# jscanvic/Scale-Equivariant-Imaging

Measured on AMD Instinct MI355X. Metric: training images/sec (256x256 crops), proposed-loss deblur, higher is better.
Workload: dtype bf16; 1 GPU; BASELINE configs[1]: deblurring Gaussian_R2 noise=5, proposed loss (SURE + scale-EI), 256x256 pairs cropped to 48 in Loss.forward, ConvolutionalModel hidden=32 scales=5; parameters=645063043, batch_per_gpu=32, global_batch=32, parallelism=dp1

## Files before the change

### include/sei_hip.h

```cpp
#ifndef SEI_HIP_H
#define SEI_HIP_H

#include <stddef.h>
#include <stdint.h>

#ifdef __cplusplus
extern "C" {
#endif

#define SEI_OK 0
#define SEI_ERR_BAD_ARG 10001
#define SEI_ERR_TOO_LARGE 10002


#define SEI_ABI_VERSION 12
int sei_abi_version(void);
int sei_build_target(char *name, int n);

int sei_event_create(void **event);
int sei_event_destroy(void *event);
int sei_event_record_external(void *event, void *stream);
int sei_stream_wait_event(void *stream, void *event);

int sei_graph_node_counts(void *graph, int *kernel_nodes, int *all_nodes);
// ... 221 lines not shown
int sei_sepmap2_small(const float *x, void *y, int out_bf16, int B, int Hi, int Wi, int Ho, int Wo, int C,
                      const float *L1, const float *R1, const float *L2, const float *R2, void *stream);
int sei_sepmap2_bf16_out16(const float *x, uint16_t *y16, int B, int Hi, int Wi, int Ho, int Wo, int C,
                           const uint16_t *packed, void *stream);

int sei_sepmap2(const float *x, float *y, int B, int Hi, int Wi, int Ho, int Wo, int C,
                const float *L1, const float *R1, const float *L2, const float *R2, float *work,
                size_t work_floats, void *stream);
int sei_sepmap2_bf16(const float *x, float *y, int B, int Hi, int Wi, int Ho, int Wo, int C, const uint16_t *packed,
                     void *stream);
int sei_sepmap2_bf16_pack(const float *L1, const float *R1, const float *L2, const float *R2, uint16_t *packed, int Hi,
                          int Wi, int Ho, int Wo, void *stream);
size_t sei_sepmap2_bf16_eligible(int B, int Hi, int Wi, int Ho, int Wo, int C);
size_t sei_sepmap2_bf16_pack_elems(int Hi, int Wi, int Ho, int Wo);
size_t sei_sepmap2_big_eligible(int B, int Hi, int Wi, int Ho, int Wo, int C);
size_t sei_sepmap2_big_pack_elems(int Hi, int Wi, int Ho, int Wo);
size_t sei_sepmap2_big_work_elems(int B, int Hi, int Wi, int Ho, int Wo, int C);
int sei_sepmap2_big_pack(const float *L1, const float *R1, const float *L2, const float *R2, uint16_t *packed,
                         int Hi, int Wi, int Ho, int Wo, void *stream);
int sei_sepmap2_big(const float *x, float *y, int B, int Hi, int Wi, int Ho, int Wo, int C, const uint16_t *packed,
                    uint16_t *work, void *stream);
int sei_sepmap2_packed(const float *x, float *y, int B, int Hi, int Wi, int Ho, int Wo, int C,
                       const float *RW, const float *LH, float *work, size_t work_floats, void *stream);

int sei_colsum_f32(const float *X, float *out, size_t M, int N, void *stream);
int sei_colsum_weighted_f32(const float *X, const float *row_weight, float *out, size_t M, int N, void *stream);

size_t sei_mlp_fused_eligible(long long M, int C);
int sei_mlp_fused_fwd(const uint16_t *h2, const uint16_t *W2, const float *b2, const uint16_t *W3, const float *b3,
                      const float *x, float res_scale, float *out, int M, int C, void *stream);
int sei_mlp_fused_bwd(const float *go, const uint16_t *h2, const uint16_t *W2, const float *b2, const uint16_t *W3T,
                      const uint16_t *W2T, float *gh2, uint16_t *go16, uint16_t *h4, uint16_t *gh3, int M, int C,
                      void *stream);

int sei_swin_attn_fwd(const float *qkv, const float *table, float *out, int B, int H, int W, int heads,
                      int head_dim, int shift, float scale, void *stream);
int sei_swin_attn_bwd(const float *qkv, const float *table, const float *dout, float *dqkv, float *dtable,
                      int B, int H, int W, int heads, int head_dim, int shift, float scale, void *stream);
int sei_swin_attn_fwd_bf16(const uint16_t *qkv, const float *table, uint16_t *out, float *lse, int B, int H, int W,
                           int heads, int shift, float scale, void *stream);
int sei_swin_attn_bwd_bf16(const uint16_t *qkv, const float *table, const uint16_t *out, const float *lse,
                           const uint16_t *dout, uint16_t *dqkv, float *dtable, int B, int H, int W, int heads,
                           int shift, float scale, void *stream);
int sei_pad_nhwc(const float *x, float *xp, int B, int H, int W, int C, int guard_rows, void *stream);
int sei_unpad_nhwc(const float *xp, const float *res, float *y, int B, int H, int W, int C, int act, void *stream);
int sei_rowscale(const float *x, const float *row_scale, const float *leaky_gate, float *y, size_t M, int N,
                 void *stream);

int sei_pack(const float *src, const int *map, void *dst, size_t n, int to_bf16, void *stream);
int sei_unpack_add(const float *src, const int *map, float *dst, size_t n, void *stream);
int sei_ln_fwd_bf16_pad(const float *x, const float *gamma, const float *beta, uint16_t *y, float *mean,
                        float *rstd, size_t rows, int C, int ldy, float eps, int ones_col, void *stream);
size_t sei_swin_partials_floats(int C);
int sei_ln_bwd_pad(const float *x, const float *gamma, const float *mean, const float *rstd, const float *gy,
                   const float *res, float *gx, float *ggamma, float *gbeta, size_t rows, int C, int ldg,
                   float *work, size_t work_floats, void *stream);
int sei_cast_pad_bf16(const float *x, const float *row_scale, uint16_t *y, float *colsum, size_t rows, int C,
                      int ldy, float *work, size_t work_floats, void *stream);
int sei_pad_nhwc_bf16(const float *x, uint16_t *xp, int B, int H, int W, int C, int Cp, int guard_rows, void *stream);
int sei_pad_nhwc_bf16_ones(const float *x, uint16_t *xp, int B, int H, int W, int C, int Cp, int guard_rows, int ones_col,
                           void *stream);
int sei_gemm_bf16nt_conv(const uint16_t *Ap, int cin_pad, const int *row_off9, const uint16_t *B, int ldb,
                         float *D32, uint16_t *D16, int M, int N, int epilogue, const float *bias, void *stream);
int sei_gemm_bf16nt_conv_unpad(const uint16_t *Ap, int cin_pad, const int *row_off9, const uint16_t *B, int ldb, float *y,
                               const float *res, int Bimg, int H, int W, int N, const float *bias, int act, void *stream);

// ... 141 lines not shown
```

### scale-equivariant-imaging_amd/_native.py

```python
import ctypes
import os

import torch

_HERE = os.path.dirname(os.path.abspath(__file__))
LIB_PATH = os.environ.get("SEI_HIP_LIBRARY") or os.path.join(_HERE, "libsei_hip.so")

SEI_REDUCE_BLOCKS = 256

_c = ctypes
_P, _I, _F, _Z, _L = _c.c_void_p, _c.c_int, _c.c_float, _c.c_size_t, _c.c_longlong

SIGNATURES = {
    "sei_abi_version": [],
    "sei_event_create": [_P],
    "sei_event_destroy": [_P],
    "sei_event_record_external": [_P, _P],
    "sei_stream_wait_event": [_P, _P],
    "sei_graph_node_counts": [_P, _P, _P],
    "sei_build_target": [_c.c_char_p, _I],
    "sei_blur_sep_circ": [_P, _P, _P, _P, _I, _I, _I, _I, _I, _I, _P],
    "sei_blur_dense_circ": [_P, _P, _P, _I, _I, _I, _I, _I, _I, _P],
    "sei_blur_dense_pad": [_P, _P, _P, _I, _I, _I, _I, _I, _I, _I, _P, _P],
    "sei_circ_filter_sep": [_P, _P, _P, _P, _I, _I, _I, _P],
# ... 50 lines not shown
    "sei_ln_fwd_bf16": [_P, _P, _P, _P, _P, _P, _Z, _I, _F, _P],
    "sei_colsum_bf16": [_P, _P, _Z, _I, _P],
    "sei_split_bf16x2": [_P, _P, _Z, _P],
    "sei_split_bf16x3": [_P, _P, _Z, _I, _P],
    "sei_gelu_f32": [_P, _P, _Z, _P],
    "sei_mul_dgelu_f32": [_P, _P, _Z, _P],
    "sei_cast_transpose_bf16": [_P, _I, _P, _P, _I, _I, _I, _P, _P],
    "sei_cast_bf16_colsum_weighted": [_P, _P, _P, _P, _I, _I, _P],
    "sei_cast_bf16_colsum_parts": [_P, _P, _P, _P, _I, _I, _P],
    "sei_gemm_bf16nt": [_P, _I, _I, _P, _I, _I, _P, _P, _I, _I, _I, _I, _P, _P, _P, _P, _P],
    "sei_gemm_bf16nt_colsum": [_P, _I, _I, _P, _I, _I, _P, _I, _I, _I, _I, _P, _P, _P],
    "sei_gemm_bf16nt_ws": [_P, _I, _I, _P, _I, _I, _P, _P, _I, _I, _I, _I, _P, _P, _P, _P, _P, _P, _Z, _I, _I, _I, _P],
    "sei_fold_many": [_P, _I, _P],
    "sei_transpose_bf16_many": [_P, _I, _P],
    "sei_gemm_bf16nt_dw2": [_P, _P, _I, _P, _P, _I, _P, _I, _I, _I, _I, _I, _P],
    "sei_gemm_bf16nt_ex": [_P, _I, _I, _P, _I, _I, _P, _P, _I, _I, _I, _I, _P, _P, _P, _P, _I, _I, _P],
    "sei_gemm_bf16nt_dw2_ex": [_P, _P, _I, _P, _P, _I, _P, _I, _I, _I, _I, _I, _I, _P],
    "sei_gemm_bf16nt_dw2_adam": [_P, _P, _I, _P, _P, _I, _P, _P, _P, _P, _P, _I, _I, _I, _I, _P],
    "sei_gemm_bf16nt_dw2_adam_ex": [_P, _P, _I, _P, _P, _I, _P, _P, _P, _P, _P, _I, _I, _I, _I, _I, _P],
    "sei_gemm_bf16nt_dw2_bf16out": [_P, _P, _I, _P, _P, _I, _P, _I, _I, _I, _I, _P],
    "sei_gemm_bf16nt_dw2_taps": [_P, _P, _I, _P, _P, _I, _P, _I, _I, _I, _I, _I, _I, _P, _L, _P],
    "sei_sepmap2": [_P, _P, _I, _I, _I, _I, _I, _I, _P, _P, _P, _P, _P, _Z, _P],
    "sei_sepmap2_big_pack": [_P, _P, _P, _P, _P, _I, _I, _I, _I, _P],
    "sei_sepmap2_big": [_P, _P, _I, _I, _I, _I, _I, _I, _P, _P, _P],
    "sei_sepmap2_packed": [_P, _P, _I, _I, _I, _I, _I, _I, _P, _P, _P, _Z, _P],
    "sei_sepmap2_bf16": [_P, _P, _I, _I, _I, _I, _I, _I, _P, _P],
    "sei_sepmap2_bf16_pack": [_P, _P, _P, _P, _P, _I, _I, _I, _I, _P],
    "sei_sepmap2_small": [_P, _P, _I, _I, _I, _I, _I, _I, _I, _P, _P, _P, _P, _P],
    "sei_sepmap2_bf16_out16": [_P, _P, _I, _I, _I, _I, _I, _I, _P, _P],
    "sei_colsum_f32": [_P, _P, _Z, _I, _P],
    "sei_colsum_weighted_f32": [_P, _P, _P, _Z, _I, _P],
    "sei_mlp_fused_fwd": [_P, _P, _P, _P, _P, _P, _F, _P, _I, _I, _P],
    "sei_mlp_fused_bwd": [_P, _P, _P, _P, _P, _P, _P, _P, _P, _P, _I, _I, _P],
    "sei_swin_attn_fwd": [_P, _P, _P, _I, _I, _I, _I, _I, _I, _F, _P],
    "sei_swin_attn_bwd": [_P, _P, _P, _P, _P, _I, _I, _I, _I, _I, _I, _F, _P],
    "sei_swin_attn_fwd_bf16": [_P, _P, _P, _P, _I, _I, _I, _I, _I, _F, _P],
    "sei_swin_attn_bwd_bf16": [_P, _P, _P, _P, _P, _P, _P, _I, _I, _I, _I, _I, _F, _P],
    "sei_pad_nhwc": [_P, _P, _I, _I, _I, _I, _I, _P],
    "sei_unpad_nhwc": [_P, _P, _P, _I, _I, _I, _I, _I, _P],
    "sei_rowscale": [_P, _P, _P, _P, _Z, _I, _P],
    "sei_pack": [_P, _P, _P, _Z, _I, _P],
    "sei_unpack_add": [_P, _P, _P, _Z, _P],
    "sei_ln_fwd_bf16_pad": [_P, _P, _P, _P, _P, _P, _Z, _I, _I, _F, _I, _P],
    "sei_ln_bwd_pad": [_P, _P, _P, _P, _P, _P, _P, _P, _P, _Z, _I, _I, _P, _Z, _P],
    "sei_cast_pad_bf16": [_P, _P, _P, _P, _Z, _I, _I, _P, _Z, _P],
    "sei_pad_nhwc_bf16": [_P, _P, _I, _I, _I, _I, _I, _I, _P],
    "sei_pad_nhwc_bf16_ones": [_P, _P, _I, _I, _I, _I, _I, _I, _I, _P],
    "sei_gemm_bf16nt_conv": [_P, _I, _P, _P, _I, _P, _P, _I, _I, _I, _P, _P],
    "sei_gemm_bf16nt_conv_unpad": [_P, _I, _P, _P, _I, _P, _P, _I, _I, _I, _I, _P, _I, _P],
    "sei_rowgemm_bf16": [_P, _I, _P, _I, _P, _I, _P, _I, _L, _I, _I, _I, _I, _P, _P, _P, _I, _P],
    "sei_rowgemm_lnbwd_bf16": [_P, _I, _P, _I, _L, _I, _P, _P, _P, _P, _P, _P, _I, _P, _P, _P, _P, _I, _P, _P, _Z, _P],
    "sei_rowgemm_dgelu_bf16": [_P, _I, _P, _I, _P, _I, _P, _I, _P, _I, _P, _I, _L, _I, _I, _P],
    "sei_rowgemm_ln_bf16": [_P, _I, _P, _I, _L, _I, _I, _P, _P, _P, _P, _P, _P, _F, _I, _P, _I, _P, _P, _P],
    "sei_rowgemm_gelu_bf16": [_P, _I, _P, _I, _P, _I, _P, _I, _L, _I, _I, _I, _P],
    "sei_tokgrad_bf16_blocks": [_P, _I, _L, _L, _P],
    "sei_tokgrad_bf16": [_P, _P, _I, _P, _P, _I, _P, _I, _I, _I, _L, _L, _P],
    "sei_dwstream_bf16_jobs": [_P, _I, _P],
    "sei_adam_fused": [_P, _P, _I, _P, _P, _Z, _F, _F, _F, _F, _F, _I, _F, _P, _P],
    "sei_adam_scalars": [_F, _F, _F, _F, _F, _I, _P, _P],
    "sei_adam_scalars_to_device": [_F, _F, _F, _F, _F, _I, _P, _P],
    "sei_sgd_fused": [_P, _P, _P, _P, _Z, _Z, _F, _F, _P, _P, _I, _P],
    "sei_sgd_penalty_finish": [_P, _Z, _P, _P],
    "sei_adam_anchor_fused": [_P, _P, _P, _P, _P, _P, _Z, _Z, _F, _F, _F, _F, _F, _I, _F, _P, _P, _I, _P],
    "sei_drunet_conv3x3": [_P, _P, _I, _I, _I, _I, _I, _I, _P, _P, _P, _P, _P],
    "sei_drunet_conv3x3_ex": [_P, _P, _I, _I, _I, _I, _I, _I, _P, _P, _P, _P, _I, _P],
    "sei_drunet_down": [_P, _P, _I, _I, _I, _I, _I, _P, _P, _P],
# ... 45 lines not shown


class TransposeJob(_c.Structure):
    _fields_ = [("src", _P), ("dst", _P), ("R", _I), ("C", _I)]


TRANSPOSE_MAX_JOBS = 16

CG_STATE_WORDS, CG_DONE, CG_ITERATIONS = 8, 3, 4


SIZE_QUERIES = {
    "sei_blur_sep_circ_lds": [_I, _I, _I, _I],
    "sei_blur_dense_pad_work_floats": [_I, _I, _I, _I, _I, _I, _I],
    "sei_resample_sepband_lds": [_I, _I, _I, _I, _I, _I, _I, _I],
    "sei_proposed_draws_max_numel": [],
    "sei_ssim_luma_work_floats": [_I, _I, _I],
    "sei_lpips_work_floats": [_I, _I, _I],
    "sei_tv_prox_work_floats": [_I, _I, _I],
    "sei_dip_work_floats": [_I, _I, _I, _I],
    "sei_dwconv7_bwd_weight_workspace": [_I, _I, _I, _I],
    "sei_dwconv7_bwd_weight_workspace_ex": [_I, _I, _I, _I, _I],
    "sei_ln_bwd_workspace": [_Z, _I],
    "sei_dwconv7_ln_fwd_launches": [_I, _I, _I, _I],
    "sei_sepmap2_bf16_eligible": [_I, _I, _I, _I, _I, _I],
    "sei_sepmap2_bf16_pack_elems": [_I, _I, _I, _I],
    "sei_sepmap2_big_eligible": [_I, _I, _I, _I, _I, _I],
    "sei_sepmap2_big_pack_elems": [_I, _I, _I, _I],
    "sei_sepmap2_big_work_elems": [_I, _I, _I, _I, _I, _I],
    "sei_swin_partials_floats": [_I],
    "sei_tokgrad_bf16_eligible": [_I, _I, _I, _I, _L, _L],
    "sei_dwstream_bf16_eligible": [_I, _I, _I, _I, _L, _L],
    "sei_mlp_fused_eligible": [_L, _I],
    "sei_rowgemm_bf16_eligible": [_L, _I, _I, _I, _I],
    "sei_rowgemm_lnbwd_bf16_eligible": [_L, _I, _I],
    "sei_rowgemm_lnbwd_work_floats": [_I],
    "sei_ln_bwd_part_offset": [_Z, _I],
    "sei_ln_bwd_part_count": [_Z, _I],
    "sei_rowgemm_dgelu_bf16_eligible": [_L, _I, _I],
    "sei_rowgemm_ln_bf16_eligible": [_L, _I, _I],
    "sei_gemm_bf16nt_plan": [_I, _I, _I, _I, _I, _I, _I, _I],
    "sei_gemm_bf16nt_plan_ws": [_I, _I, _I, _I, _I, _I, _I, _I, _Z],
    "sei_gemm_bf16nt_dw2_adam_plan": [_I, _I, _I, _I, _I],
    "sei_conv3x3_bwd_weight_parts_count": [_I, _I, _I, _I, _I, _I, _I],
    "sei_sepmap2_small_eligible": [_I, _I, _I, _I, _I, _I],
    "sei_cast_bf16_colsum_parts_count": [_I, _I],
    "sei_sgd_partials": [_Z, _Z, _I],
    "sei_adam_anchor_partials": [_Z, _Z, _I],
    "sei_drunet_work_bytes": [_I, _I, _I],
    "sei_cg_partials": [_Z],
    "sei_dps_partials": [_I, _Z],
    "sei_bm3d_ref_blocks": [_I, _I, _I],
}
ABI_VERSION = 12


class NativeLibraryError(RuntimeError):
    pass


def lib():
    global _lib
    if _lib is None:
        if not os.path.exists(LIB_PATH):
            raise NativeLibraryError(
                f"{LIB_PATH} is missing: build it with `make -C {os.path.join(_HERE, 'csrc')}` "
# ... 147 lines not shown
```

### scale-equivariant-imaging_amd/csrc/mlp128.hip

```cpp
#include "sei_common.h"

namespace {

constexpr int WAVES = 9, NT = 64 * WAVES, PX = 16 * WAVES;
constexpr int NSTAGE = 4;

template <int C>
__device__ __forceinline__ void issue_rows(char *dst, const unsigned short *m, int ht, int p, int lane) {
    int r, c;
    if constexpr (C == 128) { r = 4 * p + (lane >> 4); c = (lane & 15) ^ (r & 15); }
    else { r = 16 * p + (lane >> 2); c = (lane & 3) ^ ((-(r >> 2)) & 3); }
    __builtin_amdgcn_global_load_lds((glb_void *)(m + (size_t)(32 * ht + r) * C + 8 * c), (lds_void *)(dst + p * 1024), 16, 0, 0);
}
template <int C>
__device__ __forceinline__ void issue_cols(char *dst, const unsigned short *m, int ht, int p, int lane) {
    const int r = 16 * p + (lane >> 2), c = (lane & 3) ^ ((r >> 2) & 3);
    __builtin_amdgcn_global_load_lds((glb_void *)(m + (size_t)r * (4 * C) + 32 * ht + 8 * c), (lds_void *)(dst + p * 1024), 16, 0, 0);
}
template <int C>
__device__ __forceinline__ bf16x8 rows_frag(const char *img, int t, int ks, int l16, int lg) {
    const int r = 16 * t + l16, c = 4 * ks + lg;
    if constexpr (C == 128) return *reinterpret_cast<const bf16x8 *>(img + (16 * r + (c ^ (r & 15))) * 16);
    else return *reinterpret_cast<const bf16x8 *>(img + (4 * r + (c ^ ((-(r >> 2)) & 3))) * 16);
}
// ... 201 lines not shown
            for (int r = 0; r < 4; ++r) {
                const float h3 = hT[t][r] + bias[t][r];
                float cdf, pdf;
                sei_phi_pdf_bf16out(h3, cdf, pdf);
                const float gv = gT[t][r] * fmaf(h3, pdf, cdf);
                gT[t][r] = gv;
                a4[r] = (__bf16)(h3 * cdf);
                g4[r] = (__bf16)gv;
            }
            *reinterpret_cast<bf16x4 *>(h4p + 32 * ht + 16 * t) = a4;
            *reinterpret_cast<bf16x4 *>(g3p + 32 * ht + 16 * t) = g4;
        }
        const bf16x8 a = pack_tiles(gT[0], gT[1]);
#pragma unroll
        for (int cb = 0; cb < CB; ++cb) acc[cb] = sei_mfma16(a, wb[cb], acc[cb]);
    }
    sei_wait_vmcnt<0>();
    __syncthreads();

    constexpr int QR = C / 4, ITS = 16 * QR / 64;
    float *patch = reinterpret_cast<float *>(smem) + wave * 16 * LDP;
#pragma unroll
    for (int cb = 0; cb < CB; ++cb)
#pragma unroll
        for (int r = 0; r < 4; ++r) patch[(4 * lg + r) * LDP + 16 * cb + l16] = acc[cb][r];
    asm volatile("s_waitcnt lgkmcnt(0)" ::: "memory");
#pragma unroll
    for (int it = 0; it < ITS; ++it) {
        const int idx = it * 64 + lane, p = idx / QR, q = idx % QR;
        *reinterpret_cast<f32x4 *>(gh2 + (px0 + p) * C + 4 * q) = *reinterpret_cast<const f32x4 *>(patch + p * LDP + 4 * q);
    }
}

}

bool sei_mlp128_eligible(int M, int Cc) { return (Cc == 128 || Cc == 32) && M > 0 && M % 144 == 0; }

int sei_mlp128_fwd_launch(const uint16_t *h2, const uint16_t *W2, const float *b2, const uint16_t *W3, const float *b3,
                          const float *x, float res_scale, float *out, int M, int Cc, hipStream_t s) {
    if (Cc == 128)
        hipLaunchKernelGGL(mlp128_fwd_kernel<128>, dim3((unsigned)(M / 144)), dim3(NT), 0, s, h2, W2, b2, W3, b3, x, res_scale, out);
    else
        hipLaunchKernelGGL(mlp128_fwd_kernel<32>, dim3((unsigned)(M / 144)), dim3(NT), 0, s, h2, W2, b2, W3, b3, x, res_scale, out);
    return sei_launch_status();
}

int sei_mlp128_bwd_launch(const float *go, const uint16_t *h2, const uint16_t *W2, const float *b2, const uint16_t *W3T,
                          const uint16_t *W2T, float *gh2, uint16_t *go16, uint16_t *h4, uint16_t *gh3, int M, int Cc,
                          hipStream_t s) {
    if (Cc == 128)
        hipLaunchKernelGGL(mlp128_bwd_kernel<128>, dim3((unsigned)(M / 144)), dim3(NT), 0, s, go, h2, W2, b2, W3T, W2T, gh2,
                           go16, h4, gh3);
    else
        hipLaunchKernelGGL(mlp128_bwd_kernel<32>, dim3((unsigned)(M / 144)), dim3(NT), 0, s, go, h2, W2, b2, W3T, W2T, gh2,
                           go16, h4, gh3);
    return sei_launch_status();
}
```

### scale-equivariant-imaging_amd/csrc/mlp_fused.hip

```cpp
#include "sei_common.h"

namespace {

__device__ __forceinline__ int acc_row(int reg, int lane) { return (reg & 3) + 8 * (reg >> 2) + 4 * (lane >> 5); }
__device__ __forceinline__ bf16x8 acc_frag(const f32x16 &x, int s) {
    bf16x8 a;
#pragma unroll
    for (int e = 0; e < 8; ++e) a[e] = (__bf16)x[8 * s + e];
    return a;
}

constexpr int WAVES = 4, THREADS = 64 * WAVES;

template <int C>
struct Slices {
    static constexpr int ROW_PITCH = C * 2 + 16, COL_PITCH = 72;
    static constexpr int ROW_BYTES = 32 * ROW_PITCH, COL_BYTES = C * COL_PITCH;
    static constexpr int ROW_PIECES = 32 * C / 8, COL_PIECES = C * 4;
    static constexpr int ROW_PER_THREAD = (ROW_PIECES + THREADS - 1) / THREADS;
    static constexpr int COL_PER_THREAD = (COL_PIECES + THREADS - 1) / THREADS;
};

template <int C>
__device__ __forceinline__ void row_slice_load(const unsigned short *m, int ht, uint4 (&r)[Slices<C>::ROW_PER_THREAD]) {
// ... 292 lines not shown
                           x, res_scale, out, M);
    else
        hipLaunchKernelGGL((mlp_fwd_kernel<128, 1>), dim3(mlp_grid(M, 32 * WAVES)), dim3(THREADS), 0, s, h2, W2, b2, W3, b3,
                           x, res_scale, out, M);
    return sei_launch_status();
}

extern "C" int sei_mlp_fused_bwd(const float *go, const uint16_t *h2, const uint16_t *W2, const float *b2,
                                 const uint16_t *W3T, const uint16_t *W2T, float *gh2, uint16_t *go16, uint16_t *h4,
                                 uint16_t *gh3, int M, int C, void *stream) {
    SEI_REQUIRE(go && h2 && W2 && b2 && W3T && W2T && gh2 && go16 && h4 && gh3 && M > 0 && (C == 32 || C == 128));
    SEI_REQUIRE((((uintptr_t)go | (uintptr_t)h2 | (uintptr_t)W2 | (uintptr_t)W3T | (uintptr_t)W2T | (uintptr_t)go16) & 15) == 0 &&
                (((uintptr_t)h4 | (uintptr_t)gh3) & 7) == 0);
    hipStream_t s = (hipStream_t)stream;
    if (sei_mlp128_eligible(M, C)) {
        SEI_REQUIRE((((uintptr_t)gh2 | (uintptr_t)go) & 15) == 0);
        return sei_mlp128_bwd_launch(go, h2, W2, b2, W3T, W2T, gh2, go16, h4, gh3, M, C, s);
    }
    if (const int main = mlp128_main(M, C)) {
        SEI_REQUIRE((((uintptr_t)gh2 | (uintptr_t)go) & 15) == 0);
        if (int rc = sei_mlp128_bwd_launch(go, h2, W2, b2, W3T, W2T, gh2, go16, h4, gh3, main, C, s)) return rc;
        const size_t o = (size_t)main * C;
        go += o; h2 += o; gh2 += o; go16 += o; h4 += 4 * o; gh3 += 4 * o;
        M -= main;
    }
    if (C == 32)
        hipLaunchKernelGGL((mlp_bwd_kernel<32, 2>), dim3(mlp_grid(M, 64 * WAVES)), dim3(THREADS), 0, s, go, h2, W2, b2, W3T,
                           W2T, gh2, go16, h4, gh3, M);
    else
        hipLaunchKernelGGL((mlp_bwd_kernel<128, 1>), dim3(mlp_grid(M, 32 * WAVES)), dim3(THREADS), 0, s, go, h2, W2, b2,
                           W3T, W2T, gh2, go16, h4, gh3, M);
    return sei_launch_status();
}
```

### scale-equivariant-imaging_amd/csrc/sei_common.h

```cpp
#pragma once
#include <hip/hip_runtime.h>
#include <stdint.h>

#include "../../include/sei_hip.h"
#include "sei_mfma.h"

#define SEI_WAVE 64

typedef __attribute__((address_space(3))) void lds_void;
typedef __attribute__((address_space(1))) const void glb_void;

#define SEI_REQUIRE(cond) \
    do {                  \
        if (!(cond)) return SEI_ERR_BAD_ARG; \
    } while (0)

static inline int sei_launch_status() { return (int)hipGetLastError(); }

static inline size_t sei_ceil_div(size_t a, size_t b) { return (a + b - 1) / b; }

static inline unsigned sei_capped_grid(size_t work_items, int per_block, unsigned cap) {
    size_t g = sei_ceil_div(work_items, (size_t)per_block);
    if (g < 1) g = 1;
    if (g > cap) g = cap;
// ... 62 lines not shown
    poly = fmaf(poly, t, -0.284496736f);
    poly = fmaf(poly, t, 0.254829592f);
    const float q = 0.5f * poly * t * e;
    cdf = x >= 0.f ? 1.0f - q : q;
    pdf = 0.39894228040143267794f * e;
}
__device__ __forceinline__ float sei_gelu_bf16out(float x) {
    float cdf, pdf;
    sei_phi_pdf_bf16out(x, cdf, pdf);
    return x * cdf;
}
__device__ __forceinline__ float sei_dgelu_bf16out(float x) {
    float cdf, pdf;
    sei_phi_pdf_bf16out(x, cdf, pdf);
    return fmaf(x, pdf, cdf);
}

__device__ __forceinline__ float sei_adam_element(float pi, float gi, float &mi, float &vi, float beta1, float beta2,
                                              float eps, float wd, float step_size, float inv_bc2_sqrt) {
    if (wd != 0.f) gi = fmaf(wd, pi, gi);
    mi = mi + (gi - mi) * (1.f - beta1);
    vi = fmaf(beta2, vi, (1.f - beta2) * gi * gi);
    const float denom = sqrtf(vi) * inv_bc2_sqrt + eps;
    return pi - step_size * (mi / denom);
}


bool sei_mlp128_eligible(int M, int C);
int sei_mlp128_fwd_launch(const uint16_t *h2, const uint16_t *W2, const float *b2, const uint16_t *W3, const float *b3,
                          const float *x, float res_scale, float *out, int M, int C, hipStream_t s);
int sei_mlp128_bwd_launch(const float *go, const uint16_t *h2, const uint16_t *W2, const float *b2, const uint16_t *W3T,
                          const uint16_t *W2T, float *gh2, uint16_t *go16, uint16_t *h4, uint16_t *gh3, int M, int C,
                          hipStream_t s);

int sei_dwconv7_pipe_launch(const float *x, const float *w, const float *bias, const float *res, float res_scale,
                            float *y, int B, int H, int W, int C, int flip, hipStream_t s);
bool sei_dwconv7_pipe_eligible(const float *x, const float *w, int B, int H, int W, int C);
bool sei_dwconv7_ln_fused_eligible(const float *x, const float *w, int B, int H, int W, int C);
int sei_dwconv7_ln_fused_launch(const float *x, const float *w, const float *bias, const float *gamma,
                                const float *beta, float *h1, void *h2, int out16, float *mean, float *rstd, int B, int H,
                                int W, int C, float eps, hipStream_t s);

__attribute__((visibility("hidden"))) int sei_fold_now(const SeiFoldJob &job, hipStream_t s);
static inline SeiFoldJob sei_fold_job(int kind, const float *part, int groups, int ncol, int split, float *a, float *b,
                                      float *c) {
    SeiFoldJob J{};
    J.a = a; J.b = b; J.c = c; J.ncol = ncol; J.split = split; J.kind = kind; J.nseg = 1;
    J.part[0] = part; J.groups[0] = groups;
    return J;
}
enum { SEI_CG_FOLD_RS = 0, SEI_CG_FOLD_PAP = 1, SEI_CG_FOLD_RS_NEW = 2 };
__attribute__((visibility("hidden"))) int sei_fold_cg(const float *part, int groups, SeiCgState *state, int target, float tol,
                                                      hipStream_t s);
```

### scale-equivariant-imaging_amd/models/_ops.py

```python
import os

import torch

import _native as N
from . import _mats, _wgrad
from ._gemm import (EPI_ACCUM, EPI_BIAS, EPI_BIAS_GELU, EPI_BIAS_RES, EPI_BIAS_ROWSCALE, EPI_MUL_DGELU, EPI_NONE,
                    SPLITK_COUNTER_BYTES, SPLITK_WS_MIB, SPLITK_WS_STREAMS, _SPLITK_WS, _gemm_call, _in_forward_mode,
                    compute_dtype_scope, gemm, gemm_mixed, gemm_nt16, gemm_x3, get_compute_dtype, joint_rows,
                    own_splitk_workspace, profile_gemms, release_splitk_workspace, reset_splitk_counters, set_compute_dtype,
                    splitk_workspace)
from ._joint import JointCtx, _NotJoint, joint_ctx, walk_backward
from ._shadow import (ShadowState, _new_plain_state, _transposed16, _transposed16_cached, plain_shadow_is_current,
                      refresh_plain_shadow, set_stale_masters, shadow, split_x2, weights_updated)
from ._wgrad import (_state_for, begin_step, colsum16_into, defer_fold, direct_bf16_launches, flush_weight_grads,
                     fused_adam_launches, merged_weight_grads, note_forward, register_gradient_range,
                     set_direct_bf16_grads, set_fused_adam, set_weight_grad_merging, set_weight_grad_milestone, state_of,
                     weight_grad16, weight_grad16_group, weight_grad_views)

LN_EPS = 1e-6


def grad_of(p):
    if p.grad is None:
        view = getattr(p, "_sei_grad_view", None)
# ... 398 lines not shown
        ctx.params = (w1, b1, gamma, beta, w2, b2, w3, b3)
        ctx.twice = twice
        return out.view(B, H, W, C)

    @_in_forward_mode
    def backward(ctx, go):
        if ctx.fused:
            return ConvBlockFn16._backward_fused(ctx, go)
        x, h1, mean, rstd, h2, h3, h4 = ctx.saved_tensors
        w1, b1, gamma, beta, w2, b2, w3, b3 = ctx.params
        B, H, W, C = x.shape
        M = B * H * W
        go = go.contiguous()
        go2 = go.view(M, C)
        go16 = cast16(go2, colsum_into_=grad_of(b3))
        gh3 = torch.empty((M, 4 * C), dtype=torch.bfloat16, device=x.device)
        gemm_nt16(go16, shadow(w3), M, 4 * C, C, EPI_MUL_DGELU, out16=gh3, R1=h3, b_rmajor=True, colsum=grad_of(b2))
        weight_grad16(go16, h4, grad_of(w3).view(C, 4 * C))
        gh2 = torch.empty((M, C), dtype=torch.float32, device=x.device)
        gemm_nt16(gh3, shadow(w2), M, C, 4 * C, EPI_NONE, out32=gh2, b_rmajor=True)
        weight_grad16(gh3, h2, grad_of(w2).view(4 * C, C))
        return _convblock_tail(ctx, x, h1, mean, rstd, gh2, go)

    @staticmethod
    def _backward_fused(ctx, go):
        x, h1, mean, rstd, h2 = ctx.saved_tensors
        w1, b1, gamma, beta, w2, b2, w3, b3 = ctx.params
        B, H, W, C = x.shape
        M = B * H * W
        go = go.contiguous()
        dev = x.device
        w2_16, w3_16 = shadow(w2), shadow(w3)
        gh2 = torch.empty((M, C), dtype=torch.float32, device=dev)
        go16 = torch.empty((M, C), dtype=torch.bfloat16, device=dev)
        h4 = torch.empty((M, 4 * C), dtype=torch.bfloat16, device=dev)
        gh3 = torch.empty((M, 4 * C), dtype=torch.bfloat16, device=dev)
        w3t, w2t = _transposed16_cached(w3, w3_16), _transposed16_cached(w2, w2_16)
        args = (go.data_ptr(), h2.data_ptr(), w2_16.data_ptr(), b2.data_ptr(), w3t.data_ptr(), w2t.data_ptr(),
                gh2.data_ptr(), go16.data_ptr(), h4.data_ptr(), gh3.data_ptr(), M, C)
        _gemm_call(4.0 * M * 4 * C * C, "sei_mlp_fused_bwd", *args)
        if _wgrad.DWSTREAM and N.lib().sei_dwstream_bf16_eligible(C, 4 * C, C, 4 * C, M, 0):
            weight_grad16(go16, h4, grad_of(w3).view(C, 4 * C), bias=grad_of(b3))
            weight_grad16(gh3, h2, grad_of(w2).view(4 * C, C), bias=grad_of(b2))
        else:
            colsum_into(grad_of(b3), go.view(M, C))
            colsum16_into(grad_of(b2), gh3)
            weight_grad16(go16, h4, grad_of(w3).view(C, 4 * C))
            weight_grad16(gh3, h2, grad_of(w2).view(4 * C, C))
        return _convblock_tail(ctx, x, h1, mean, rstd, gh2, go)

    @staticmethod
    def joint_ctx(c1, c2, rec):
        if c1.fused != c2.fused or c1.twice != c2.twice:
            raise _NotJoint()
        return JointCtx(c1, [rec.joint(a, b) for a, b in zip(c1.saved_tensors, c2.saved_tensors)])

    @staticmethod
    def walk(ctx, g, skips):
        return ConvBlockFn16.backward(ctx, g)[0]


class DownsampleFn16(torch.autograd.Function):

    @staticmethod
    def forward(ctx, x, gamma, beta, w, b, rate, with_skip=False):
        ctx.dtype = get_compute_dtype()
        ctx.set_materialize_grads(False)
        x = _nhwc(x)
        h, mean, rstd = layer_norm(x.view(-1, x.shape[-1]), gamma, beta)
        B, H, W, C, Co, fwd, bwd, Ho, Wo = _resample_prologue("down", x, w, rate)
        u = sepmap2_16(h.view(B, H, W, C), fwd, Ho, Wo, out16=True)
        Mo = B * Ho * Wo
        s = _mats.constant_response("down", H, W, rate, x.device, B)
        u16 = u.view(Mo, C) if u.dtype == torch.bfloat16 else cast16(u.view(Mo, C))
# ... 131 lines not shown
```

### scale-equivariant-imaging_amd/models/_wgrad.py

```python
import collections
import os
import weakref

import torch

import _native as N
from . import _gemm
from ._gemm import EPI_ACCUM, EPI_NONE, _gemm_call, gemm_mixed, gemm_nt16

TOKEN_STREAMING = os.environ.get("SEI_SWIN_TILED") != "1"

DWSTREAM = os.environ.get("SEI_NO_DWSTREAM") != "1"

DEFERRED_FOLDS = os.environ.get("SEI_NO_DEFERRED_FOLDS") != "1"

SINK_ADAM, SINK_BF16 = "adam", "direct16"
_SINKS = {SINK_ADAM: ("sei_gemm_bf16nt_dw2_adam", "fused optimizer step"),
          SINK_BF16: ("sei_gemm_bf16nt_dw2_bf16out", "bf16 gradients written into the exchange buffer")}

_Queued = collections.namedtuple("_Queued", "job operands grad flops")


def _segments(pairs):
    (g1, x1), (g2, x2) = pairs[0], pairs[-1]
    return g1, x1, g2, x2, g1.shape[0], (g2.shape[0] if len(pairs) == 2 else 0)


def colsum16_into(acc, x16):
    M, Nn = x16.shape
    N.call("sei_colsum_bf16", x16.data_ptr(), acc.data_ptr(), M, Nn)


def _dwstream_ok(grad2d, pairs):
    if not DWSTREAM or not grad2d.is_cuda or grad2d.dim() != 2 or grad2d.dtype != torch.float32 or len(pairs) > 2 \
            or grad2d.stride(1) != 1:
        return False
    Np, Kp = grad2d.shape
    for gy, x in pairs:
        if not (gy.dtype == x.dtype == torch.bfloat16 and gy.is_contiguous() and x.is_contiguous()
                and gy.dim() == 2 and x.dim() == 2 and gy.shape[1] == Np and x.shape[1] == Kp and gy.shape[0] == x.shape[0]):
            return False
    return N.lib().sei_dwstream_bf16_eligible(Np, Kp, Np, Kp, *_segments(pairs)[4:]) != 0


class GradRecord:
# ... 181 lines not shown
            return False
        Np, Kp = grad2d.shape
        g1, x1, g2, x2, K1, K2 = _segments(pairs)
        job = N.DwStreamJob(g1.data_ptr(), g2.data_ptr(), x1.data_ptr(), x2.data_ptr(), Np, Kp, Np, Kp, grad2d.data_ptr(),
                            grad2d.stride(0), 0, K1, K2, N.ptr(bias))
        self.dwjobs.append(_Queued(job, (g1, x1, g2, x2, bias), grad2d, per_row * (K1 + K2)))
        if len(self.dwjobs) == N.DWSTREAM_MAX_JOBS or not self.queue_flush():
            self.flush_dwstream()
        return True

    def flush_dwstream(self):
        jobs, self.dwjobs = self.dwjobs, []
        if not jobs:
            return
        arr = (N.DwStreamJob * len(jobs))(*[q.job for q in jobs])
        _gemm_call(sum(q.flops for q in jobs), "sei_dwstream_bf16_jobs", arr, len(jobs))

    def defer_fold(self, a, b, c, ncol, split, kind, work, offset, groups):
        if not self.queue_flush():
            return False
        key = a.data_ptr()
        meta = (N.ptr(b), N.ptr(c), int(ncol), int(split), int(kind))
        job = self.folds.get(key)
        if job is not None and (job["meta"] != meta or len(job["segs"]) == 3):
            self.flush_folds()
            job = None
        if job is None:
            if len(self.folds) == N.FOLD_MAX_JOBS:
                self.flush_folds()
            job = self.folds[key] = {"meta": meta, "segs": []}
        job["segs"].append((work, work.data_ptr() + 4 * int(offset), int(groups)))
        return True

    def flush_folds(self):
        jobs, self.folds = self.folds, {}
        if not jobs:
            return
        arr = (N.FoldJob * len(jobs))()
        for j, (a_ptr, job) in zip(arr, jobs.items()):
            b_ptr, c_ptr, ncol, split, kind = job["meta"]
            j.a, j.b, j.c, j.ncol, j.split, j.kind, j.nseg = a_ptr, b_ptr, c_ptr, ncol, split, kind, len(job["segs"])
            for k, (_, ptr, groups) in enumerate(job["segs"]):
                j.part[k] = ptr
                j.groups[k] = groups
        N.call("sei_fold_many", arr, len(jobs))

    def queue_flush(self):
        if not self.flush_queued:
            try:
                torch.autograd.Variable._execution_engine.queue_callback(self.flush)
            except RuntimeError:
                return False
            self.flush_queued = True
        return True

    def flush(self):
        self.flush_queued = False
        parked, self.parked = self.parked, {}
        for entry in parked.values():
            if isinstance(entry, list):
                self.launch_group([entry])
            else:
                self.launch(entry[2], [entry[:2]])
        self.flush_dwstream()
        self.flush_folds()

# ... 85 lines not shown


def flush_weight_grads(owner=None):
    state_of(owner).flush()


def weight_grad16(gy16, x16, grad2d, flops_per_row=None, tap_rows=None, bias=None):
    key = grad2d.data_ptr()
    st = _state_for(key)
    rec = st.meet(grad2d, flops_per_row, tap_rows)
    if bias is not None:
        rec.bias = bias
    split = _gemm._JOINT_SPLIT
    if split is not None and tap_rows is None:
        M1 = gy16.shape[0] * split[0] // (split[0] + split[1])
        rec.arrivals += 2
        st.launch(grad2d, [(gy16[:M1], x16[:M1]), (gy16[M1:], x16[M1:])])
        return
    rec.arrivals += 1
    st.arrive(key, rec.arrivals, (gy16, x16, grad2d), lambda entries: st.launch(grad2d, [e[:2] for e in entries]))


def weight_grad16_group(items):
    items = list(items)
    head = items[0][2].data_ptr()
    st = _state_for(head)
    for _, _, grad2d, fpr in items:
        st.meet(grad2d, fpr).arrivals += 1
    st.arrive(("group", head), st.records[head].arrivals, items, st.launch_group)


def defer_fold(a, b, c, ncol, split, kind, work, offset, groups):
    return DEFERRED_FOLDS and _state_for(a.data_ptr()).defer_fold(a, b, c, ncol, split, kind, work, offset, groups)
```

Baseline: 2766 images/s.

## Fuse MLP weight-gradient accumulation into the C=32 fused MLP backward kernel

Adds a new HIP kernel for the C=32 MLP backward that computes the input gradient and also accumulates the W2/W3/bias weight gradients in registers via MFMA over LDS-resident tiles. Each workgroup writes per-group partial sums, which are later reduced through the existing deferred fold mechanism. This removes the bf16 intermediates (go16, h4, gh3) and the two separate streamed weight-gradient GEMMs, cutting memory traffic and launches. In exchange it adds heavy LDS use, a partial-sum buffer per call, and a complex eligibility path with a grid capped at 256 groups.

```diff
diff --git a/include/sei_hip.h b/include/sei_hip.h
--- a/include/sei_hip.h
+++ b/include/sei_hip.h
@@ -277,6 +277,10 @@
 int sei_mlp_fused_bwd(const float *go, const uint16_t *h2, const uint16_t *W2, const float *b2, const uint16_t *W3T,
                       const uint16_t *W2T, float *gh2, uint16_t *go16, uint16_t *h4, uint16_t *gh3, int M, int C,
                       void *stream);
+size_t sei_mlp_fused_bwd_wgrad_eligible(long long M, int C);
+size_t sei_mlp_fused_bwd_wgrad_parts_count(long long M, int C, int max_groups);
+int sei_mlp_fused_bwd_wgrad(const float *go, const uint16_t *h2, const uint16_t *W2, const float *b2, const uint16_t *W3T,
+                            const uint16_t *W2T, float *gh2, float *parts, int M, int C, int max_groups, void *stream);
 
 int sei_swin_attn_fwd(const float *qkv, const float *table, float *out, int B, int H, int W, int heads,
                       int head_dim, int shift, float scale, void *stream);
diff --git a/scale-equivariant-imaging_amd/_native.py b/scale-equivariant-imaging_amd/_native.py
--- a/scale-equivariant-imaging_amd/_native.py
+++ b/scale-equivariant-imaging_amd/_native.py
@@ -106,6 +106,7 @@
     "sei_colsum_weighted_f32": [_P, _P, _P, _Z, _I, _P],
     "sei_mlp_fused_fwd": [_P, _P, _P, _P, _P, _P, _F, _P, _I, _I, _P],
     "sei_mlp_fused_bwd": [_P, _P, _P, _P, _P, _P, _P, _P, _P, _P, _I, _I, _P],
+    "sei_mlp_fused_bwd_wgrad": [_P, _P, _P, _P, _P, _P, _P, _P, _I, _I, _I, _P],
     "sei_swin_attn_fwd": [_P, _P, _P, _I, _I, _I, _I, _I, _I, _F, _P],
     "sei_swin_attn_bwd": [_P, _P, _P, _P, _P, _I, _I, _I, _I, _I, _I, _F, _P],
     "sei_swin_attn_fwd_bf16": [_P, _P, _P, _P, _I, _I, _I, _I, _I, _F, _P],
@@ -217,6 +218,8 @@
     "sei_tokgrad_bf16_eligible": [_I, _I, _I, _I, _L, _L],
     "sei_dwstream_bf16_eligible": [_I, _I, _I, _I, _L, _L],
     "sei_mlp_fused_eligible": [_L, _I],
+    "sei_mlp_fused_bwd_wgrad_eligible": [_L, _I],
+    "sei_mlp_fused_bwd_wgrad_parts_count": [_L, _I, _I],
     "sei_rowgemm_bf16_eligible": [_L, _I, _I, _I, _I],
     "sei_rowgemm_lnbwd_bf16_eligible": [_L, _I, _I],
     "sei_rowgemm_lnbwd_work_floats": [_I],
diff --git a/scale-equivariant-imaging_amd/csrc/mlp128.hip b/scale-equivariant-imaging_amd/csrc/mlp128.hip
--- a/scale-equivariant-imaging_amd/csrc/mlp128.hip
+++ b/scale-equivariant-imaging_amd/csrc/mlp128.hip
@@ -257,6 +257,162 @@
     }
 }
 
+constexpr int WG_IMG = 64 * 32, WG_STAGE = 3 * WG_IMG, WG_WEIGHTS = 4 * WG_STAGE;
+constexpr int WG_TILE = PX * 64;
+constexpr int WG_LB2 = WG_WEIGHTS, WG_GO = WG_LB2 + 512, WG_H2 = WG_GO + WG_TILE, WG_HG = WG_H2 + WG_TILE;
+constexpr int WG_LDS = WG_HG + 4 * WG_TILE;
+constexpr int WG_NW = 32 * 128 + 128 * 32, WG_NB = 128 + 32;
+
+__device__ __forceinline__ int tile_off(int row, int col) {
+    return row * 64 + ((((col >> 4) ^ (row >> 2)) & 1) << 5) + (col & 15) * 2;
+}
+__device__ __forceinline__ int tile_tr_lane(int l16, int lg) { return tile_off(4 * lg + (l16 >> 2), 4 * (l16 & 3)); }
+__device__ __forceinline__ v4s tile_tr(const char *img, int tr_lane, int blk, int s) {
+    return __builtin_amdgcn_ds_read_tr16_b64_v4i16(
+        (__attribute__((address_space(3))) v4s *)(img + (tr_lane ^ (32 * blk)) + 1024 * s));
+}
+__device__ __forceinline__ f32x4 mfma16k16(v4s a, v4s b, f32x4 c) {
+    return __builtin_amdgcn_mfma_f32_16x16x16bf16_1k(a, b, c, 0, 0, 0);
+}
+
+__global__ __launch_bounds__(NT) __attribute__((amdgpu_waves_per_eu(5))) void mlp32_bwd_wgrad_kernel(const float *__restrict__ go, const unsigned short *__restrict__ h2,
+                                                             const unsigned short *__restrict__ W2,
+                                                             const float *__restrict__ b2,
+                                                             const unsigned short *__restrict__ W3T,
+                                                             const unsigned short *__restrict__ W2T,
+                                                             float *__restrict__ gh2, float *__restrict__ parts, int ntiles) {
+    constexpr int C = 32, H4 = 4 * C, NSLICE = 4, CB = 2, LDP = C;
+    __shared__ __attribute__((aligned(1024))) char smem[WG_LDS];
+    float *lb2 = reinterpret_cast<float *>(smem + WG_LB2);
+    const int tid = threadIdx.x, lane = tid & 63, l16 = lane & 15, lg = lane >> 4;
+    const int wave = __builtin_amdgcn_readfirstlane(tid >> 6);
+
+    for (int q = wave; q < 6 * NSLICE; q += WAVES) {
+        const int ht = q / 6, im = (q % 6) >> 1, p = q & 1;
+        char *dst = smem + ht * WG_STAGE + im * WG_IMG;
+        if (im == 0) issue_rows<C>(dst, W2, ht, p, lane);
+        else if (im == 1) issue_rows<C>(dst, W3T, ht, p, lane);
+        else issue_cols<C>(dst, W2T, ht, p, lane);
+    }
+    if (tid < H4) lb2[tid] = b2[tid];
+    const int row = 16 * wave + l16;
+    const int tr_lane = tile_tr_lane(l16, lg);
+    const int kind = wave >> 2, bi = (wave >> 1) & 1, bj = wave & 1;
+    auto ones = [&](int sel) {
+        const short one = (l16 >> 2) == sel ? (short)0x3F80 : (short)0;
+        return v4s{one, one, one, one};
+    };
+    f32x4 wacc[NSLICE];
+#pragma unroll
+    for (int ht = 0; ht < NSLICE; ++ht) wacc[ht] = f32x4{0.f, 0.f, 0.f, 0.f};
+    asm volatile("s_waitcnt vmcnt(0)" ::: "memory");
+    __syncthreads();
+
+#pragma unroll 1
+    for (int tile = blockIdx.x; tile < ntiles; tile += gridDim.x) {
+        const size_t px0 = (size_t)tile * PX + 16 * wave;
+        const size_t o = (px0 + l16) * C + 8 * lg;
+        const bf16x8 f = *reinterpret_cast<const bf16x8 *>(h2 + o);
+        const f32x4 ga = *reinterpret_cast<const f32x4 *>(go + o), gb = *reinterpret_cast<const f32x4 *>(go + o + 4);
+        const bf16x8 g = pack_tiles(ga, gb);
+        __syncthreads();
+        *reinterpret_cast<bf16x8 *>(smem + WG_GO + tile_off(row, 8 * lg)) = g;
+        *reinterpret_cast<bf16x8 *>(smem + WG_H2 + tile_off(row, 8 * lg)) = f;
+        f32x4 acc[CB];
+#pragma unroll
+        for (int cb = 0; cb < CB; ++cb) acc[cb] = f32x4{0.f, 0.f, 0.f, 0.f};
+#pragma unroll 1
+        for (int ht = 0; ht < NSLICE; ++ht) {
+            const char *st = smem + ht * WG_STAGE;
+            char *hg = smem + WG_HG + (ht & 1) * 2 * WG_TILE;
+            f32x4 hT[2], gT[2];
+#pragma unroll
+            for (int t = 0; t < 2; ++t) {
+                const bf16x8 wa = rows_frag<C>(st, t, 0, l16, lg), wg = rows_frag<C>(st + WG_IMG, t, 0, l16, lg);
+                hT[t] = sei_mfma16(wa, f, f32x4{0.f, 0.f, 0.f, 0.f});
+                gT[t] = sei_mfma16(wg, g, f32x4{0.f, 0.f, 0.f, 0.f});
+            }
+            f32x4 bias[2];
+#pragma unroll
+            for (int t = 0; t < 2; ++t) bias[t] = *reinterpret_cast<const f32x4 *>(lb2 + 32 * ht + 16 * t + 4 * lg);
+#pragma unroll
+            for (int t = 0; t < 2; ++t) {
+                bf16x4 a4, g4;
+#pragma unroll
+                for (int r = 0; r < 4; ++r) {
+                    const float h3 = hT[t][r] + bias[t][r];
+                    float cdf, pdf;
+                    sei_phi_pdf_bf16out(h3, cdf, pdf);
+                    const float gv = gT[t][r] * fmaf(h3, pdf, cdf);
+                    gT[t][r] = gv;
+                    a4[r] = (__bf16)(h3 * cdf);
+                    g4[r] = (__bf16)gv;
+                }
+                *reinterpret_cast<bf16x4 *>(hg + tile_off(row, 16 * t + 4 * lg)) = a4;
+                *reinterpret_cast<bf16x4 *>(hg + WG_TILE + tile_off(row, 16 * t + 4 * lg)) = g4;
+            }
+            __builtin_amdgcn_sched_barrier(0);
+            const bf16x8 a = pack_tiles(gT[0], gT[1]);
+#pragma unroll
+            for (int cb = 0; cb < CB; ++cb) acc[cb] = sei_mfma16(a, cols_frag(st + 2 * WG_IMG, cb, l16, lg), acc[cb]);
+            __syncthreads();
+            if (wave < 8) {
+                const char *ia = kind == 0 ? smem + WG_GO : hg + WG_TILE, *ib = kind == 0 ? hg : smem + WG_H2;
+                const int ba = kind == 0 ? bi : bj, bb = kind == 0 ? bj : bi;
+#pragma unroll
+                for (int s = 0; s < WAVES; ++s) {
+                    if (s % 3 == 0) __builtin_amdgcn_sched_barrier(0);
+                    wacc[0] = mfma16k16(tile_tr(ia, tr_lane, ba, s), tile_tr(ib, tr_lane, bb, s), wacc[0]);
+                }
+            } else {
+#pragma unroll
+                for (int j = 0; j < 2; ++j)
+#pragma unroll
+                    for (int s = 0; s < WAVES; ++s)
+                        wacc[0] = mfma16k16(ones(j), tile_tr(hg + WG_TILE, tr_lane, j, s), wacc[0]);
+                if (ht == 0) {
+#pragma unroll
+                    for (int i = 0; i < 2; ++i)
+#pragma unroll
+                        for (int s = 0; s < WAVES; ++s)
+                            wacc[0] = mfma16k16(ones(2 + i), tile_tr(smem + WG_GO, tr_lane, i, s), wacc[0]);
+                }
+            }
+            const f32x4 w0 = wacc[0];
+            wacc[0] = wacc[1]; wacc[1] = wacc[2]; wacc[2] = wacc[3]; wacc[3] = w0;
+        }
+        constexpr int QR = C / 4, ITS = 16 * QR / 64;
+        float *patch = reinterpret_cast<float *>(smem + WG_HG) + wave * 16 * LDP;
+#pragma unroll
+        for (int cb = 0; cb < CB; ++cb)
+#pragma unroll
+            for (int r = 0; r < 4; ++r) patch[(4 * lg + r) * LDP + 16 * cb + l16] = acc[cb][r];
+        asm volatile("s_waitcnt lgkmcnt(0)" ::: "memory");
+#pragma unroll
+        for (int it = 0; it < ITS; ++it) {
+            const int idx = it * 64 + lane, p = idx / QR, q = idx % QR;
+            *reinterpret_cast<f32x4 *>(gh2 + (px0 + p) * C + 4 * q) = *reinterpret_cast<const f32x4 *>(patch + p * LDP + 4 * q);
+        }
+    }
+
+    float *pw = parts + (size_t)blockIdx.x * WG_NW;
+    float *pb = parts + (size_t)gridDim.x * WG_NW + (size_t)blockIdx.x * WG_NB;
+    if (wave < 8) {
+#pragma unroll
+        for (int ht = 0; ht < NSLICE; ++ht)
+#pragma unroll
+            for (int r = 0; r < 4; ++r) {
+                if (kind == 0) pw[(16 * bi + 4 * lg + r) * H4 + 32 * ht + 16 * bj + l16] = wacc[ht][r];
+                else pw[C * H4 + (32 * ht + 16 * bj + 4 * lg + r) * C + 16 * bi + l16] = wacc[ht][r];
+            }
+    } else {
+#pragma unroll
+        for (int ht = 0; ht < NSLICE; ++ht)
+            if (lg < 2) pb[32 * ht + 16 * lg + l16] = wacc[ht][0];
+        if (lg >= 2) pb[H4 + 16 * (lg - 2) + l16] = wacc[0][0];
+    }
+}
+
 }
 
 bool sei_mlp128_eligible(int M, int Cc) { return (Cc == 128 || Cc == 32) && M > 0 && M % 144 == 0; }
@@ -281,3 +437,15 @@
                            go16, h4, gh3);
     return sei_launch_status();
 }
+
+int sei_mlp32_wgrad_groups(long long M, int max_groups) {
+    const long long tiles = M / 144, cap = max_groups > 0 && max_groups < 256 ? max_groups : 256;
+    return (int)(tiles < cap ? tiles : cap);
+}
+
+int sei_mlp32_bwd_wgrad_launch(const float *go, const uint16_t *h2, const uint16_t *W2, const float *b2, const uint16_t *W3T,
+                               const uint16_t *W2T, float *gh2, float *parts, int M, int max_groups, hipStream_t s) {
+    hipLaunchKernelGGL(mlp32_bwd_wgrad_kernel, dim3((unsigned)sei_mlp32_wgrad_groups(M, max_groups)), dim3(NT), 0, s, go, h2, W2,
+                       b2, W3T, W2T, gh2, parts, M / 144);
+    return sei_launch_status();
+}
diff --git a/scale-equivariant-imaging_amd/csrc/mlp_fused.hip b/scale-equivariant-imaging_amd/csrc/mlp_fused.hip
--- a/scale-equivariant-imaging_amd/csrc/mlp_fused.hip
+++ b/scale-equivariant-imaging_amd/csrc/mlp_fused.hip
@@ -348,3 +348,20 @@
                            W3T, W2T, gh2, go16, h4, gh3, M);
     return sei_launch_status();
 }
+
+extern "C" size_t sei_mlp_fused_bwd_wgrad_eligible(long long M, int C) {
+    return C == 32 && M > 0 && M < (1ll << 31) && M % 144 == 0 ? 1 : 0;
+}
+
+extern "C" size_t sei_mlp_fused_bwd_wgrad_parts_count(long long M, int C, int max_groups) {
+    return sei_mlp_fused_bwd_wgrad_eligible(M, C) ? (size_t)sei_mlp32_wgrad_groups(M, max_groups) : 0;
+}
+
+extern "C" int sei_mlp_fused_bwd_wgrad(const float *go, const uint16_t *h2, const uint16_t *W2, const float *b2,
+                                       const uint16_t *W3T, const uint16_t *W2T, float *gh2, float *parts, int M, int C,
+                                       int max_groups, void *stream) {
+    SEI_REQUIRE(go && h2 && W2 && b2 && W3T && W2T && gh2 && parts && max_groups >= 0 && sei_mlp_fused_bwd_wgrad_eligible(M, C));
+    SEI_REQUIRE((((uintptr_t)go | (uintptr_t)h2 | (uintptr_t)W2 | (uintptr_t)W3T | (uintptr_t)W2T | (uintptr_t)gh2) & 15) == 0 &&
+                ((uintptr_t)parts & 3) == 0);
+    return sei_mlp32_bwd_wgrad_launch(go, h2, W2, b2, W3T, W2T, gh2, parts, M, max_groups, (hipStream_t)stream);
+}
diff --git a/scale-equivariant-imaging_amd/csrc/sei_common.h b/scale-equivariant-imaging_amd/csrc/sei_common.h
--- a/scale-equivariant-imaging_amd/csrc/sei_common.h
+++ b/scale-equivariant-imaging_amd/csrc/sei_common.h
@@ -118,6 +118,9 @@
 int sei_mlp128_bwd_launch(const float *go, const uint16_t *h2, const uint16_t *W2, const float *b2, const uint16_t *W3T,
                           const uint16_t *W2T, float *gh2, uint16_t *go16, uint16_t *h4, uint16_t *gh3, int M, int C,
                           hipStream_t s);
+int sei_mlp32_wgrad_groups(long long M, int max_groups);
+int sei_mlp32_bwd_wgrad_launch(const float *go, const uint16_t *h2, const uint16_t *W2, const float *b2, const uint16_t *W3T,
+                               const uint16_t *W2T, float *gh2, float *parts, int M, int max_groups, hipStream_t s);
 
 int sei_dwconv7_pipe_launch(const float *x, const float *w, const float *bias, const float *res, float res_scale,
                             float *y, int B, int H, int W, int C, int flip, hipStream_t s);
diff --git a/scale-equivariant-imaging_amd/models/_ops.py b/scale-equivariant-imaging_amd/models/_ops.py
--- a/scale-equivariant-imaging_amd/models/_ops.py
+++ b/scale-equivariant-imaging_amd/models/_ops.py
@@ -454,14 +454,23 @@
         dev = x.device
         w2_16, w3_16 = shadow(w2), shadow(w3)
         gh2 = torch.empty((M, C), dtype=torch.float32, device=dev)
+        w3t, w2t = _transposed16_cached(w3, w3_16), _transposed16_cached(w2, w2_16)
+        streamed = _wgrad.DWSTREAM and N.lib().sei_dwstream_bf16_eligible(C, 4 * C, C, 4 * C, M, 0) != 0
+        grads = (grad_of(w3).view(C, 4 * C), grad_of(w2).view(4 * C, C), grad_of(b3), grad_of(b2))
+        groups = _wgrad.fused_mlp_wgrad_groups(grads, M, C) if streamed else 0
+        if groups:
+            parts = torch.empty(groups * (8 * C * C + 5 * C), dtype=torch.float32, device=dev)
+            _gemm_call(8.0 * M * 4 * C * C, "sei_mlp_fused_bwd_wgrad", go.data_ptr(), h2.data_ptr(), w2_16.data_ptr(),
+                       b2.data_ptr(), w3t.data_ptr(), w2t.data_ptr(), gh2.data_ptr(), parts.data_ptr(), M, C, 0)
+            _wgrad.fused_mlp_wgrad_fold(parts, groups, grads, M)
+            return _convblock_tail(ctx, x, h1, mean, rstd, gh2, go)
         go16 = torch.empty((M, C), dtype=torch.bfloat16, device=dev)
         h4 = torch.empty((M, 4 * C), dtype=torch.bfloat16, device=dev)
         gh3 = torch.empty((M, 4 * C), dtype=torch.bfloat16, device=dev)
-        w3t, w2t = _transposed16_cached(w3, w3_16), _transposed16_cached(w2, w2_16)
         args = (go.data_ptr(), h2.data_ptr(), w2_16.data_ptr(), b2.data_ptr(), w3t.data_ptr(), w2t.data_ptr(),
                 gh2.data_ptr(), go16.data_ptr(), h4.data_ptr(), gh3.data_ptr(), M, C)
         _gemm_call(4.0 * M * 4 * C * C, "sei_mlp_fused_bwd", *args)
-        if _wgrad.DWSTREAM and N.lib().sei_dwstream_bf16_eligible(C, 4 * C, C, 4 * C, M, 0):
+        if streamed:
             weight_grad16(go16, h4, grad_of(w3).view(C, 4 * C), bias=grad_of(b3))
             weight_grad16(gh3, h2, grad_of(w2).view(4 * C, C), bias=grad_of(b2))
         else:
diff --git a/scale-equivariant-imaging_amd/models/_wgrad.py b/scale-equivariant-imaging_amd/models/_wgrad.py
--- a/scale-equivariant-imaging_amd/models/_wgrad.py
+++ b/scale-equivariant-imaging_amd/models/_wgrad.py
@@ -11,6 +11,8 @@
 TOKEN_STREAMING = os.environ.get("SEI_SWIN_TILED") != "1"
 
 DWSTREAM = os.environ.get("SEI_NO_DWSTREAM") != "1"
+
+MLP_WGRAD = os.environ.get("SEI_NO_MLP_WGRAD") != "1"
 
 DEFERRED_FOLDS = os.environ.get("SEI_NO_DEFERRED_FOLDS") != "1"
 
@@ -258,6 +260,30 @@
         job["segs"].append((work, work.data_ptr() + 4 * int(offset), int(groups)))
         return True
 
+    def fused_mlp_wgrad_groups(self, grads, M, C):
+        if not (MLP_WGRAD and DWSTREAM and DEFERRED_FOLDS) or any(g is None for g in grads):
+            return 0
+        for g in grads:
+            rec = self.records.get(g.data_ptr())
+            if not (g.is_cuda and g.dtype == torch.float32 and g.is_contiguous()) or _state_for(g.data_ptr()) is not self \
+                    or (rec is not None and rec.sink is not None) or self.in_early_release_range(g.data_ptr()) \
+                    or (self.store and g.numel() >= self.store_min):
+                return 0
+        groups = N.lib().sei_mlp_fused_bwd_wgrad_parts_count(M, C, 0)
+        return groups if groups and self.queue_flush() else 0
+
+    def fused_mlp_wgrad_fold(self, parts, groups, grads, M, joint):
+        gw3, gw2, gb3, gb2 = grads
+        for g in (gw3, gw2):
+            self.meet(g).arrivals += 2 if joint else 1
+
+        def fold():
+            ok = self.defer_fold(gw3, gw2, None, gw3.numel() + gw2.numel(), gw3.numel(), N.FOLD_SPLIT, parts, 0, groups)
+            ok = ok and self.defer_fold(gb2, gb3, None, gb2.numel() + gb3.numel(), gb2.numel(), N.FOLD_SPLIT, parts,
+                                        groups * (gw3.numel() + gw2.numel()), groups)
+            assert ok, "fused_mlp_wgrad_groups promised a running backward pass"
+        self._launch([gw3.data_ptr(), gw2.data_ptr()], joint and self.whole_step(2) and M % 8 == 0, fold)
+
     def flush_folds(self):
         jobs, self.folds = self.folds, {}
         if not jobs:
@@ -409,3 +435,11 @@
 
 def defer_fold(a, b, c, ncol, split, kind, work, offset, groups):
     return DEFERRED_FOLDS and _state_for(a.data_ptr()).defer_fold(a, b, c, ncol, split, kind, work, offset, groups)
+
+
+def fused_mlp_wgrad_groups(grads, M, C):
+    return 0 if grads[0] is None else _state_for(grads[0].data_ptr()).fused_mlp_wgrad_groups(grads, M, C)
+
+
+def fused_mlp_wgrad_fold(parts, groups, grads, M):
+    _state_for(grads[0].data_ptr()).fused_mlp_wgrad_fold(parts, groups, grads, M, _gemm._JOINT_SPLIT is not None)
```

Result: no change. 2782 images/s (median of 6 runs) (+0.6%).
